# FluidInference/FluidAudio

Hardware: NVIDIA H100
Metric: audio-hours/s (higher is better)
Workload: dtype f32

## Files before the change

fluidaudio_b200/csrc/fa_common.cuh:

```cuda
#pragma once

#include <cstddef>
#include <cstdint>

#if defined(__CUDACC__)
#include <atomic>
#include <cstdio>
#include <memory>
#include <type_traits>
#include <utility>
#include <cuda_runtime.h>
#define FA_HD __host__ __device__ __forceinline__
#else
#define FA_HD inline
#endif

enum : int {
    FA_OK = 0,
    FA_INVALID_ARGUMENT = 1,
    FA_INDEX_OVERFLOW = 2,
    FA_OUTPUT_TOO_SMALL = 3,
    FA_ALLOCATION_FAILURE = 4,
    FA_RUNTIME_ERROR = 5,
    FA_NO_DEVICE = 6,
    FA_CUDA_ERROR = 7,
    FA_UNSUPPORTED = 8,
    FA_UNKNOWN_ERROR = 255,
};

namespace fa {

void set_error(const char *fmt, ...);
const char *last_error();

struct Carver {
    char *base = nullptr;
    size_t off = 0;
    template <typename T> T *take(size_t count) {
        off = (off + 255) & ~size_t(255);
        T *p = reinterpret_cast<T *>(base + off);
        off += count * sizeof(T);
        return p;
    }
};

#if defined(__CUDACC__)
struct CudaStatus {
    int code;
    template <typename T> operator T() const { return static_cast<T>(code); }
};
inline CudaStatus cuda_failure(cudaError_t e, const char *expr, const char *file, int line) {
    set_error("%s failed: %s (%s:%d)", expr, cudaGetErrorString(e), file, line);
    (void)cudaGetLastError();
    return CudaStatus{e == cudaErrorMemoryAllocation ? FA_ALLOCATION_FAILURE : FA_CUDA_ERROR};
}
#define FA_CUDA_TRY(expr)                                                                 \
    do {                                                                                  \
        const cudaError_t e__ = (expr);                                                   \
        if (e__ != cudaSuccess) return fa::cuda_failure(e__, #expr, __FILE__, __LINE__); \
    } while (0)

template <bool Pinned> struct CudaFree {
    void operator()(void *p) const { Pinned ? cudaFreeHost(p) : cudaFree(p); }
};

template <typename T, bool Pinned> class GrowBuffer {
  public:
    GrowBuffer() = default;
    GrowBuffer(GrowBuffer &&o) noexcept : p_(std::move(o.p_)), cap_(std::exchange(o.cap_, 0)) {}
    GrowBuffer &operator=(GrowBuffer &&o) noexcept {
        p_ = std::move(o.p_);
        cap_ = std::exchange(o.cap_, 0);
        return *this;
    }
    int grow(size_t bytes) {
        if (bytes <= cap_) return FA_OK;
        p_.reset();
        cap_ = 0;
        void *q = nullptr;
        const cudaError_t e = Pinned ? cudaMallocHost(&q, bytes) : cudaMalloc(&q, bytes);
        if (e != cudaSuccess) {
            char what[64];
            std::snprintf(what, sizeof(what), "%s(%zu bytes)", Pinned ? "cudaMallocHost" : "cudaMalloc", bytes);
            return cuda_failure(e, what, __FILE__, __LINE__);
        }
        p_.reset(q);
        cap_ = bytes;
        return FA_OK;
    }
    T *data() const { return static_cast<T *>(p_.get()); }
    size_t capacity() const { return cap_; }

  private:
    std::unique_ptr<void, CudaFree<Pinned>> p_;
    size_t cap_ = 0;
};
template <typename T = void> using DeviceBuffer = GrowBuffer<T, false>;
template <typename T = void> using PinnedBuffer = GrowBuffer<T, true>;

template <typename T, bool Pinned, typename Layout>
int carve_arena(GrowBuffer<T, Pinned> &buf, Layout &&layout, size_t slack = 0) {
    Carver size{nullptr};
    layout(size);
    const int st = buf.grow(size.off + slack);
    if (st != FA_OK) return st;
    Carver c{static_cast<char *>(static_cast<void *>(buf.data()))};
    layout(c);
    return FA_OK;
}

template <typename A, typename B>
int grow_slots(int slots, int grown, cudaStream_t stream, DeviceBuffer<A> &a, size_t a_slot, DeviceBuffer<B> &b,
               size_t b_slot) {
    DeviceBuffer<A> na;
    DeviceBuffer<B> nb;
    int st = na.grow((size_t)grown * a_slot * sizeof(A));
    if (st == FA_OK) st = nb.grow((size_t)grown * b_slot * sizeof(B));
    if (st != FA_OK) return st;
    if (slots) {
        FA_CUDA_TRY(cudaMemcpyAsync(na.data(), a.data(), (size_t)slots * a_slot * sizeof(A), cudaMemcpyDeviceToDevice, stream));
        FA_CUDA_TRY(cudaMemcpyAsync(nb.data(), b.data(), (size_t)slots * b_slot * sizeof(B), cudaMemcpyDeviceToDevice, stream));
        FA_CUDA_TRY(cudaStreamSynchronize(stream));
    }
    a = std::move(na);
    b = std::move(nb);
    return FA_OK;
}

struct StreamDestroy {
    void operator()(cudaStream_t s) const { cudaStreamDestroy(s); }
};
struct EventDestroy {
    void operator()(cudaEvent_t e) const { cudaEventDestroy(e); }
};
struct Stream : std::unique_ptr<std::remove_pointer_t<cudaStream_t>, StreamDestroy> {
    operator cudaStream_t() const { return get(); }
    int create(unsigned flags = cudaStreamNonBlocking) {
        cudaStream_t s = nullptr;
        FA_CUDA_TRY(cudaStreamCreateWithFlags(&s, flags));
        reset(s);
        return FA_OK;
    }
};
struct Event : std::unique_ptr<std::remove_pointer_t<cudaEvent_t>, EventDestroy> {
    operator cudaEvent_t() const { return get(); }
    int create(unsigned flags = cudaEventDefault) {
        cudaEvent_t e = nullptr;
        FA_CUDA_TRY(cudaEventCreateWithFlags(&e, flags));
        reset(e);
        return FA_OK;
    }
};

template <typename T = void> struct UploadStage {
    PinnedBuffer<T> host;
    DeviceBuffer<T> device;
    Event uploaded;
    bool in_flight = false;

    int reserve(size_t bytes) {
        if (in_flight) {
            FA_CUDA_TRY(cudaEventSynchronize(uploaded));
            in_flight = false;
        }
        const int st = device.grow(bytes);
        return st != FA_OK ? st : host.grow(bytes);
    }
    int upload(size_t bytes, cudaStream_t stream) {
        if (!uploaded) {
            const int st = uploaded.create(cudaEventDisableTiming);
            if (st != FA_OK) return st;
        }
        FA_CUDA_TRY(cudaMemcpyAsync(device.data(), host.data(), bytes, cudaMemcpyHostToDevice, stream));
        FA_CUDA_TRY(cudaEventRecord(uploaded, stream));
        in_flight = true;
        return FA_OK;
    }
};

extern std::atomic<long long> g_launches;

template <typename... Params, typename... Args>
cudaError_t launch(void (*kernel)(Params...), dim3 grid, dim3 block, size_t smem, cudaStream_t stream, Args &&...args) {
    kernel<<<grid, block, smem, stream>>>(std::forward<Args>(args)...);
    g_launches.fetch_add(1, std::memory_order_relaxed);
    return cudaGetLastError();
}

template <typename T> struct kernel_param { using type = T; };
template <typename... Params>
cudaError_t launch_cooperative(void (*kernel)(Params...), dim3 grid, dim3 block, size_t smem, cudaStream_t stream,
                               typename kernel_param<Params>::type... args) {
    void *argv[] = {&args...};
    const cudaError_t e =
        cudaLaunchCooperativeKernel(reinterpret_cast<const void *>(kernel), grid, block, argv, smem, stream);
    g_launches.fetch_add(1, std::memory_order_relaxed);
    return e != cudaSuccess ? e : cudaGetLastError();
}

inline int sm90_device_props(int dev, cudaDeviceProp &prop) {
    FA_CUDA_TRY(cudaGetDeviceProperties(&prop, dev));
    if (prop.major != 9) {
        set_error("fluidaudio_b200 requires an sm_90a device, found sm_%d%d", prop.major, prop.minor);
        return FA_NO_DEVICE;
    }
    return FA_OK;
}

__device__ __forceinline__ float2 fadd2_rn(float2 a, float2 b) { return make_float2(__fadd_rn(a.x, b.x), __fadd_rn(a.y, b.y)); }
__device__ __forceinline__ float2 fmul2_rn(float2 a, float2 b) { return make_float2(__fmul_rn(a.x, b.x), __fmul_rn(a.y, b.y)); }
__device__ __forceinline__ float2 ffma2_rn(float2 a, float2 b, float2 c) {
    return make_float2(__fmaf_rn(a.x, b.x, c.x), __fmaf_rn(a.y, b.y, c.y));
}
#endif

}
```

fluidaudio_b200/csrc/mel_kernels.cu:

```cuda
#include "mel_core.cuh"
#include "mel_plan.h"

#include <cuda_runtime.h>
#include <algorithm>
#include <cmath>
#include <vector>

namespace fa {
namespace mel {

__device__ __forceinline__ uint32_t smem_u32(const void *p) { return (uint32_t)__cvta_generic_to_shared(p); }

__device__ __forceinline__ void mbar_init(uint64_t *bar, uint32_t count) {
    asm volatile("mbarrier.init.shared::cta.b64 [%0], %1;" ::"r"(smem_u32(bar)), "r"(count));
}
__device__ __forceinline__ void mbar_expect_tx(uint64_t *bar, uint32_t bytes) {
    asm volatile("mbarrier.arrive.expect_tx.shared::cta.b64 _, [%0], %1;" ::"r"(smem_u32(bar)), "r"(bytes) : "memory");
}
__device__ __forceinline__ void mbar_arrive(uint64_t *bar) {
    asm volatile("mbarrier.arrive.shared::cta.b64 _, [%0];" ::"r"(smem_u32(bar)) : "memory");
}
__device__ __forceinline__ bool mbar_try_wait(uint64_t *bar, uint32_t parity) {
    uint32_t ok;
    asm volatile(
        "{\n\t"
        ".reg .pred p;\n\t"
        "mbarrier.try_wait.parity.shared::cta.b64 p, [%1], %2;\n\t"
        "selp.u32 %0, 1, 0, p;\n\t"
        "}"
        : "=r"(ok)
        : "r"(smem_u32(bar)), "r"(parity)
        : "memory");
    return ok != 0;
}
__device__ __forceinline__ void mbar_wait(uint64_t *bar, uint32_t parity) {
    while (!mbar_try_wait(bar, parity)) {
    }
}
__device__ __forceinline__ void bulk_g2s(void *dst, const void *src, uint32_t bytes, uint64_t *bar) {
    asm volatile("cp.async.bulk.shared::cluster.global.mbarrier::complete_tx::bytes [%0], [%1], %2, [%3];" ::"r"(
                     smem_u32(dst)),
                 "l"(src), "r"(bytes), "r"(smem_u32(bar))
                 : "memory");
}
__device__ __forceinline__ void fence_proxy_async() { asm volatile("fence.proxy.async.shared::cta;" ::: "memory"); }

struct TileGeom {
    int unit;
    long long f0;
    int nf;
    long long a0;
    long long base;
    long long gs, ge;
};

__device__ __forceinline__ const MelUnit &unit_at(const MelLaunch &P, int idx) { return P.inline_unit ? P.unit0 : P.units[idx]; }

__device__ __forceinline__ TileGeom tile_geom(const MelLaunch &P, int tile) {
    int lo = 0, hi = P.inline_unit ? 0 : P.num_units - 1;
    while (lo < hi) {
        const int mid = (lo + hi + 1) >> 1;
        if (P.units[mid].tile_begin <= tile) lo = mid; else hi = mid - 1;
    }
    const MelUnit &u = P.inline_unit ? P.unit0 : P.units[lo];
    TileGeom g;
    g.unit = lo;
    g.f0 = u.frame_begin + (long long)kTileFrames * (tile - u.tile_begin);
    const long long rem = u.frame_begin + u.frame_count - g.f0;
    g.nf = rem < kTileFrames ? (int)rem : kTileFrames;
    g.a0 = g.f0 * P.hop - P.pad;
    const long long need0 = g.a0 - 1;
    g.base = (need0 >= 0) ? (need0 & ~3LL) : -(((-need0) + 3) & ~3LL);
    long long ge = (g.a0 + P.pt_len + 3) & ~3LL;
    const long long n4 = u.n & ~3LL;
    if (ge > n4) ge = n4;
    g.gs = g.base < 0 ? 0 : g.base;
    g.ge = ge;
    if (!P.use_tma) g.ge = g.gs;
    return g;
}

struct TileInfo {
    TileGeom g;
    long long audio_off, n, out_off, out_stride;
    float last;
    int pad_;
};
__device__ __forceinline__ void make_tile_info(const MelLaunch &P, int tile, TileInfo &ti) {
    ti.g = tile_geom(P, tile);
    const MelUnit &u = unit_at(P, ti.g.unit);
    ti.audio_off = u.audio_off;
    ti.n = u.n;
    ti.out_off = u.out_off;
    ti.out_stride = u.out_stride;
    ti.last = u.last;
}

template <int kWarps, typename V, int kLayout>
__global__ void __launch_bounds__(kWarps * 32, 2) mel512_kernel(const MelLaunch P) {
    constexpr int kF = vtraits<V>::kFrames;
    extern __shared__ __align__(128) unsigned char smem[];
    float *raw0 = reinterpret_cast<float *>(smem);
    float *raw1 = raw0 + P.raw_cap;
    float *ptile = raw1 + P.raw_cap;
    cpxv<V> *fftbuf = reinterpret_cast<cpxv<V> *>(ptile + P.pt_cap);
    float *power = reinterpret_cast<float *>(fftbuf + kWarps * kFftPad);
    float *otile = power + (kTileFrames / 2) * kPairStride;
    const int ot_stride = P.ot_stride;
    float *fbw = otile + kTileFrames * ot_stride;
    int4 *fbmeta = reinterpret_cast<int4 *>(fbw + P.fb_cap);
    uint64_t *bars = reinterpret_cast<uint64_t *>(fbmeta + P.n_slots);
    TileInfo *tinfo = reinterpret_cast<TileInfo *>(bars + 2);

    const int tid = threadIdx.x, lane = tid & 31, warp = tid >> 5;

    if (tid == 0) {
        mbar_init(&bars[0], 1);
        mbar_init(&bars[1], 1);
        asm volatile("fence.mbarrier_init.release.cluster;" ::: "memory");
    }
    for (int i = tid; i < P.fb_nnz; i += kWarps * 32) fbw[i] = P.fb_w[i];
    for (int i = tid; i < P.n_slots; i += kWarps * 32) fbmeta[i] = P.fb_slots[i];
    for (int i = tid; i < (kTileFrames / 2) * kPairStride; i += kWarps * 32) power[i] = 0.0f;
    const LaneTables<V> T = reinterpret_cast<const LaneTables<V> *>(P.lane_tab)[lane];
    __syncthreads();

    cpxv<V> *buf = fftbuf + warp * kFftPad;

    auto issue = [&](int tile, int buf, TileInfo &slot) {
        make_tile_info(P, tile, slot);
        const TileGeom &g = slot.g;
        float *dst = buf ? raw1 : raw0;
        if (g.ge > g.gs) {
            const uint32_t bytes = (uint32_t)((g.ge - g.gs) * 4);
            mbar_expect_tx(&bars[buf], bytes);
            bulk_g2s(dst + (g.gs - g.base), P.audio + slot.audio_off + g.gs, bytes, &bars[buf]);
        } else {
            mbar_arrive(&bars[buf]);
        }
    };

    auto preemphasize = [&](const TileInfo &u, const float *raw) {
        const TileGeom &g = u.g;
        const float a = P.preemph;
        const bool interior = g.a0 >= 1 && g.a0 - 1 >= g.gs && g.a0 + P.pt_len <= g.ge && g.a0 + P.pt_len <= u.n;
        if (interior) {
            const float *src = raw + (g.a0 - g.base);
            if (((g.a0 - g.base) & 3) == 0 && (P.pt_len & 3) == 0) {
                const float4 *s4 = reinterpret_cast<const float4 *>(src);
                float4 *d4 = reinterpret_cast<float4 *>(ptile);
                for (int q = tid; q < (P.pt_len >> 2); q += kWarps * 32) {
                    const float4 x = s4[q];
                    float4 y = x;
                    const float prev = src[4 * q - 1];
                    if (a != 0.0f) {
                        y.x = preemph_rest(x.x, prev, a);
                        y.y = preemph_rest(x.y, x.x, a);
                        y.z = preemph_rest(x.z, x.y, a);
                        y.w = preemph_rest(x.w, x.z, a);
                    }
                    d4[q] = y;
                }
            } else if (a == 0.0f) {
                for (int t = tid; t < P.pt_len; t += kWarps * 32) ptile[t] = src[t];
            } else {
                for (int t = tid; t < P.pt_len; t += kWarps * 32) ptile[t] = preemph_rest(src[t], src[t - 1], a);
            }
        } else {
            const float *gaudio = P.audio + u.audio_off;
            auto sample = [&](long long i) -> float {
                if (i >= g.gs && i < g.ge) return raw[i - g.base];
                if (i < 0) return u.last;
                return __ldg(gaudio + i);
            };
            for (int t = tid; t < P.pt_len; t += kWarps * 32) {
                const long long i = g.a0 + t;
                float v = 0.0f;
                if (i >= 0 && i < u.n) {
                    const float x = sample(i);
                    if (a == 0.0f) v = x;
                    else if (i == 0) v = preemph_first(x, u.last, a);
                    else v = preemph_rest(x, sample(i - 1), a);
                }
                ptile[t] = v;
            }
        }
    };
    auto copy_out = [&](float *dst, int total) {
        if (P.out_vec4) {
            float4 *d4 = reinterpret_cast<float4 *>(dst);
            for (int q = tid; q < (total >> 2); q += kWarps * 32) {
                const int e = 4 * q;
                const int row = (int)__umulhi((unsigned)e, P.inv_n_mels);
                d4[q] = *reinterpret_cast<const float4 *>(otile + e + 4 * row);
            }
        } else {
            const int row_pad = ot_stride - P.n_mels;
            for (int idx = tid; idx < total; idx += kWarps * 32) {
                const int fi = P.n_mels == 1 ? idx : (int)__umulhi((unsigned)idx, P.inv_n_mels);
                dst[idx] = otile[idx + fi * row_pad];
            }
        }
    };

    const int first = blockIdx.x, stride = gridDim.x;
    if (first >= P.total_tiles) return;
    if (tid == 0) {
        issue(first, 0, tinfo[0]);
        if (first + stride < P.total_tiles) issue(first + stride, 1, tinfo[1]);
    }
    __syncthreads();
    mbar_wait(&bars[0], 0);
    preemphasize(tinfo[0], raw0);
    __syncthreads();
    float *pending_dst = nullptr;
    int pending_total = 0;
    int it = 0, slot = 0;
    for (int tile = first; tile < P.total_tiles; tile += stride, ++it, slot = slot == 2 ? 0 : slot + 1) {
        const TileInfo &u = tinfo[slot];
        const int nf = u.g.nf;

        if (pending_dst) copy_out(pending_dst, pending_total);
        for (int fi = warp * kF; fi < nf; fi += kWarps * kF) {
            const float *pf = ptile + fi * P.hop;
            V re[8], im[8];
            if (P.mid_full) pass1<true>(lane, pf, P.hop, T, buf); else pass1<false>(lane, pf, P.hop, T, buf);
            __syncwarp();
            pass2_load(lane, buf, re, im);
            __syncwarp();
            pass2_store(lane, T, re, im, buf);
            __syncwarp();
            pass3_post(lane, buf, T, power + (fi >> 1) * kPairStride + (fi & 1));
            __syncwarp();
        }
        __syncthreads();

        const int next = tile + stride;
        const int slot1 = slot == 2 ? 0 : slot + 1, slot2 = slot1 == 2 ? 0 : slot1 + 1;
        if (tid == 0 && next + stride < P.total_tiles) {
            fence_proxy_async();
            issue(next + stride, it & 1, tinfo[slot2]);
        }
        {
            constexpr int kPairs = kTileFrames / 2, kGroup = 32 / kPairs;
            const int pl = lane % kPairs, mg = lane / kPairs;
            const float *prow = power + pl * kPairStride;
            float *orow = otile + (2 * pl) * ot_stride;
            float *gout = kLayout == 1 ? P.out + u.out_off + u.g.f0 + 2 * pl : nullptr;
            for (int slot = warp * kGroup + mg; slot < P.n_slots; slot += kWarps * kGroup) {
                const int4 md = fbmeta[slot];
                const float2 a2 = mel_dot_pairs(reinterpret_cast<const float4 *>(prow + 2 * md.x),
                                                reinterpret_cast<const float4 *>(fbw + md.z), md.y);
                const float v0 = log_value(a2.x, P.log_floor, P.log_clamped, P.log_normal),
                            v1 = log_value(a2.y, P.log_floor, P.log_clamped, P.log_normal);
                const int m = md.w;
                if (m < 0) continue;
                if (kLayout == 0) {
                    orow[m] = v0;
                    orow[ot_stride + m] = v1;
                } else {
                    float *g = gout + (long long)m * u.out_stride;
                    if (2 * pl < nf) g[0] = v0;
                    if (2 * pl + 1 < nf) g[1] = v1;
                }
            }
        }
        if (kLayout == 0) {
            pending_dst = P.out + u.out_off + u.g.f0 * P.n_mels;
            pending_total = nf * P.n_mels;
        }
        if (next < P.total_tiles) {
            const int nb = (it + 1) & 1;
            mbar_wait(&bars[nb], (uint32_t)((it + 1) >> 1) & 1u);
            preemphasize(tinfo[slot1], nb ? raw1 : raw0);
        }
        __syncthreads();
    }
    if (pending_dst) copy_out(pending_dst, pending_total);
}


struct GenericParams {
    int n_fft, log2n, bins, prow;
    const cpxd *tw;
    int warps;
    float spectrum_power;
    float log_mean, log_std;
};

template <bool kReflect, int kSpectrum, bool kAffine>
__global__ void __launch_bounds__(256) mel_generic_kernel(const MelLaunch P, const GenericParams G) {
    extern __shared__ __align__(16) unsigned char smem[];
    cpxd *tw = reinterpret_cast<cpxd *>(smem);
    cpxd *fft = tw + G.n_fft / 2;
    float *power = reinterpret_cast<float *>(fft + (size_t)G.warps * G.n_fft);
    float *win = power + (size_t)G.warps * G.prow;
    const int tid = threadIdx.x, lane = tid & 31, warp = tid >> 5, nthreads = G.warps * 32;
    for (int i = tid; i < G.n_fft / 2; i += nthreads) tw[i] = G.tw[i];
    for (int i = tid; i < G.n_fft; i += nthreads) win[i] = P.in_tab[i] ? P.win_tab[i] : 0.0f;
    for (int i = tid; i < G.warps * G.prow; i += nthreads) power[i] = 0.0f;
    __syncthreads();
    cpxd *buf = fft + (size_t)warp * G.n_fft;
    float *prow = power + (size_t)warp * G.prow;
    const float a = P.preemph;
    for (int tile = blockIdx.x; tile < P.total_tiles; tile += gridDim.x) {
        const TileGeom g = tile_geom(P, tile);
        const MelUnit u = unit_at(P, g.unit);
        const float *x = P.audio + u.audio_off;
        for (int fi = warp; fi < g.nf; fi += G.warps) {
            const long long f = g.f0 + fi;
            const long long base = f * P.hop - P.pad;
            for (int j = lane; j < G.n_fft; j += 32) {
                const long long i = base + j;
                float v = 0.0f;
                if (kReflect) {
                    if (u.n > 0 && P.in_tab[j]) v = __fmul_rn(__ldg(x + reflect_index(i, u.n)), win[j]);
                } else if (i >= 0 && i < u.n && P.in_tab[j]) {
                    const float xi = __ldg(x + i);
                    if (a == 0.0f) v = xi;
                    else if (i == 0) v = preemph_first(xi, u.last, a);
                    else v = preemph_rest(xi, __ldg(x + i - 1), a);
                    v = __fmul_rn(v, win[j]);
                }
                cpxd z;
                z.x = (double)v;
                z.y = 0.0;
                buf[__brev((unsigned)j) >> (32 - G.log2n)] = z;
            }
            __syncwarp();
            for (int s = 0; s < G.log2n; ++s) {
                const int half = 1 << s, step = G.n_fft >> (s + 1);
                for (int t = lane; t < G.n_fft / 2; t += 32) {
                    const int j = t & (half - 1);
                    const int ia = ((t >> s) << (s + 1)) + j, ib = ia + half;
                    const cpxd w = tw[j * step], zb = buf[ib], za = buf[ia];
                    const double tr = zb.x * w.x - zb.y * w.y, ti = zb.x * w.y + zb.y * w.x;
                    cpxd o;
                    o.x = za.x - tr;
                    o.y = za.y - ti;
                    buf[ib] = o;
                    o.x = za.x + tr;
                    o.y = za.y + ti;
                    buf[ia] = o;
                }
                __syncwarp();
            }
            for (int b = lane; b < G.bins; b += 32) {
                const float xr = (float)buf[b].x, xi = (float)buf[b].y;
                const float pw = __fadd_rn(__fmul_rn(xr, xr), __fmul_rn(xi, xi));
                if (kSpectrum == kSpecPower) prow[b] = 4.0f * pw;
                else if (kSpectrum == kSpecMagnitude) prow[b] = __fsqrt_rn(pw);
                else prow[b] = powf(__fsqrt_rn(pw), G.spectrum_power);
            }
            __syncwarp();
            for (int m = lane; m < P.n_mels; m += 32) {
                const int lo = P.fb_lo[m], nq = (P.fb_hi[m] - lo) >> 2;
                float v = log_value(mel_dot_quads(reinterpret_cast<const float4 *>(prow + lo),
                                                  reinterpret_cast<const float4 *>(P.fb_w + P.fb_off[m]), nq),
                                    P.log_floor, P.log_clamped);
                if (kAffine) v = __fdiv_rn(__fsub_rn(v, G.log_mean), G.log_std);
                if (P.layout == 0) P.out[u.out_off + f * P.n_mels + m] = v;
                else P.out[u.out_off + (long long)m * u.out_stride + f] = v;
            }
            __syncwarp();
        }
    }
}

static constexpr int kCtasPerSm = 2;

typedef void (*Mel512Kernel)(const MelLaunch);
template <typename V> static Mel512Kernel mel512_variant(int layout) {
    return layout == FA_MEL_TIME_MAJOR ? mel512_kernel<kWarpsPerCta, V, FA_MEL_TIME_MAJOR>
                                       : mel512_kernel<kWarpsPerCta, V, FA_MEL_MEL_MAJOR>;
}
static Mel512Kernel mel512_variant(int precision, int layout) {
    return precision == FA_MEL_PRECISION_F64 ? mel512_variant<double>(layout) : mel512_variant<f32x2>(layout);
}

typedef void (*GenericKernel)(const MelLaunch, const GenericParams);
template <bool R, int S> static GenericKernel generic_variant(bool affine) {
    return affine ? mel_generic_kernel<R, S, true> : mel_generic_kernel<R, S, false>;
}
template <bool R> static GenericKernel generic_variant(int spectrum, bool affine) {
    return spectrum == kSpecPower ? generic_variant<R, kSpecPower>(affine)
                                  : (spectrum == kSpecMagnitude ? generic_variant<R, kSpecMagnitude>(affine)
                                                                : generic_variant<R, kSpecGeneral>(affine));
}
static GenericKernel generic_variant(bool reflect, int spectrum, bool affine) {
    return reflect ? generic_variant<true>(spectrum, affine) : generic_variant<false>(spectrum, affine);
}

static int placement_of(int mode) { return mode == FA_MEL_LEGACY_COMPUTE ? 1 : 0; }
static int window_offset(const MelConfig &c, int placement) { return placement == 1 ? 0 : (c.n_fft - c.win_length) / 2; }

static_assert(sizeof(MelSlot) == sizeof(int4) && offsetof(MelSlot, mel) == offsetof(int4, w), "MelSlot is an int4");

template <typename T, typename U> static int upload_table(DeviceBuffer<T> &b, const std::vector<U> &v) {
    const int st = b.grow(std::max<size_t>(1, v.size()) * sizeof(U));
    if (st != FA_OK) return st;
    if (!v.empty()) FA_CUDA_TRY(cudaMemcpy(b.data(), v.data(), v.size() * sizeof(U), cudaMemcpyHostToDevice));
    return FA_OK;
}

int MelPlan::init(const MelConfig &c) {
    cfg = c;
    if (cfg.pad_to < 1) cfg.pad_to = 1;
    if (cfg.n_mels <= 0 || cfg.hop_length <= 0 || cfg.win_length <= 0 || cfg.n_fft <= 0 || cfg.sample_rate <= 0) {
        fa::set_error("mel config: all sizes must be positive");
        return FA_INVALID_ARGUMENT;
    }
    const bool pow2 = cfg.n_fft >= 32 && cfg.n_fft <= 4096 && (cfg.n_fft & (cfg.n_fft - 1)) == 0;
    if (!pow2 || cfg.win_length > cfg.n_fft || cfg.n_mels > 512 || cfg.hop_length > 65536) {
        fa::set_error("mel config unsupported by the sm_90a kernels: need nFFT a power of two in 32..4096, win <= nFFT, "
                      "nMels <= 512 (got nFFT=%d hop=%d win=%d nMels=%d)",
                      cfg.n_fft, cfg.hop_length, cfg.win_length, cfg.n_mels);
        return FA_UNSUPPORTED;
    }
    if (const char *why = check_ex_config(cfg)) {
        fa::set_error("mel ex config: %s", why);
        return FA_INVALID_ARGUMENT;
    }
    const int spectrum = spectrum_kind(cfg.spectrum_power);
    generic = cfg.n_fft != kNfft || (cfg.hop_length & 1) || cfg.hop_length > 1024 || cfg.reflect() ||
              spectrum != kSpecPower || cfg.affine();
    const int n_fft = cfg.n_fft, bins = n_fft / 2 + 1;
    build_tables(cfg, window, filterbank);
    const MelBands bands = pack_bands(filterbank, cfg.n_mels, bins);
    fb_nnz = bands.nnz;
    n_slots = (int)bands.slots.size();

    int dev = 0;
    FA_CUDA_TRY(cudaGetDevice(&dev));
    cudaDeviceProp prop;
    int st = sm90_device_props(dev, prop);
    if (st != FA_OK) return st;
    num_sms = prop.multiProcessorCount;

    if (!generic) {
        pt_len = (kTileFrames - 1) * cfg.hop_length + kNfft;
        pt_cap = (pt_len + 31) & ~31;
        raw_cap = (pt_len + 1 + 3 + 3 + 31) & ~31;
        fb_cap = (fb_nnz + 3) & ~3;
        smem_bytes = sizeof(float) * ((size_t)2 * raw_cap + pt_cap + 0 +
                                      (size_t)(kTileFrames / 2) * kPairStride + (size_t)kTileFrames * (cfg.n_mels + 4) + fb_cap) +
                     sizeof(cpxd) * (size_t)kWarpsPerCta * kFftPad + sizeof(int) * 4 * (size_t)n_slots + 8 +
                     2 * sizeof(uint64_t) + 3 * sizeof(TileInfo) + 16;
        if (smem_bytes > (size_t)prop.sharedMemPerBlockOptin) {
            generic = true;
            pt_len = pt_cap = raw_cap = fb_cap = 0;
        }
    }

    std::vector<float> win_tab;
    std::vector<uint8_t> in_tab;
    for (int pl = 0; pl < 2; ++pl) {
        place_window(window, n_fft, window_offset(cfg, pl), win_tab, in_tab);
        st = upload_table(d_win_tab_mode[pl], win_tab);
        if (st == FA_OK) st = upload_table(d_in_tab_mode[pl], in_tab);
        if (st != FA_OK) return st;
        if (!generic) {
            std::vector<LaneTables<double>> t64(32);
            std::vector<LaneTables<f32x2>> t32(32);
            for (int l = 0; l < 32; ++l) {
                load_lane_tables(l, win_tab.data(), in_tab.data(), t64[l]);
                load_lane_tables(l, win_tab.data(), in_tab.data(), t32[l]);
            }
            st = upload_table(d_lane_tab[pl][FA_MEL_PRECISION_F64], t64);
            if (st == FA_OK) st = upload_table(d_lane_tab[pl][FA_MEL_PRECISION_F32], t32);
            if (st != FA_OK) return st;
        }
    }
    st = upload_table(d_fb_w, pack_weights(filterbank, bands, bins, !generic, spectrum == kSpecPower ? 0.25f : 1.0f));
    if (st == FA_OK) st = upload_table(d_fb_slots, bands.slots);
    if (st == FA_OK) st = upload_table(d_fb_lo, bands.lo);
    if (st == FA_OK) st = upload_table(d_fb_hi, bands.hi);
    if (st == FA_OK) st = upload_table(d_fb_off, bands.off);
    for (auto &s : streams)
        if (st == FA_OK) st = s.create();
    if (st != FA_OK) return st;
    if (generic) {
        std::vector<cpxd> tw(n_fft / 2);
        for (int k = 0; k < n_fft / 2; ++k) tw[k] = unit_root(k, n_fft);
        st = upload_table(d_generic_tw, tw);
        if (st != FA_OK) return st;
        generic_prow = ((bins + 3) & ~3) + 4;
        int log2n = 0;
        while ((1 << log2n) < n_fft) ++log2n;
        generic_log2n = log2n;
        const size_t fixed = (size_t)(n_fft / 2) * sizeof(cpxd) + (size_t)n_fft * sizeof(float);
        const size_t per_warp = (size_t)n_fft * sizeof(cpxd) + (size_t)generic_prow * sizeof(float);
        generic_warps = (int)std::min<size_t>(8, ((size_t)prop.sharedMemPerBlockOptin - fixed - 1024) / per_warp);
        if (generic_warps < 1) {
            fa::set_error("mel config: nFFT %d does not fit shared memory", n_fft);
            return FA_UNSUPPORTED;
        }
        smem_bytes = fixed + per_warp * generic_warps;
        for (const bool r : {false, cfg.reflect()})
            FA_CUDA_TRY(cudaFuncSetAttribute(generic_variant(r, spectrum, cfg.affine()),
                                             cudaFuncAttributeMaxDynamicSharedMemorySize, (int)smem_bytes));
        return FA_OK;
    }
    for (const int precision : {FA_MEL_PRECISION_F64, FA_MEL_PRECISION_F32})
        for (const int layout : {FA_MEL_TIME_MAJOR, FA_MEL_MEL_MAJOR})
            FA_CUDA_TRY(cudaFuncSetAttribute(mel512_variant(precision, layout), cudaFuncAttributeMaxDynamicSharedMemorySize,
                                             (int)smem_bytes));
    return FA_OK;
}

long long MelPlan::frame_count(long long n, int mode, long long expected) const {
    long long computed;
    if (mode == FA_MEL_PAD_CENTER) computed = 1 + (n + 2 * (long long)(cfg.n_fft / 2) - cfg.win_length) / cfg.hop_length;
    else if (mode == FA_MEL_PAD_PREPADDED) computed = std::max<long long>(0, (n - cfg.n_fft) / cfg.hop_length + 1);
    else computed = 1 + (n - cfg.win_length) / cfg.hop_length;
    return expected >= 0 ? expected : computed;
}

int MelPlan::ensure_staging(size_t audio_floats, size_t out_floats) {
    const int st = d_audio.grow(audio_floats * sizeof(float));
    return st != FA_OK ? st : d_out.grow(out_floats * sizeof(float));
}

int MelPlan::ensure_events(size_t count) {
    while (events.size() < count) {
        Event e;
        const int st = e.create(cudaEventDisableTiming);
        if (st != FA_OK) return st;
        events.push_back(std::move(e));
    }
    return FA_OK;
}

static int tiles_of(long long frames) { return (int)((frames + kTileFrames - 1) / kTileFrames); }

int number_tiles(MelUnit *u, int count) {
    int tiles = 0;
    for (int i = 0; i < count; ++i) {
        u[i].tile_begin = tiles;
        tiles += tiles_of(u[i].frame_count);
    }
    return tiles;
}

int MelPlan::launch(const MelUnit *d_u, const MelUnit *h_u, int count, bool inline_unit, const float *d_audio_base,
                    float *d_out_base, int mode, int layout, cudaStream_t stream) {
    const int total_tiles = count > 0 ? h_u[count - 1].tile_begin + tiles_of(h_u[count - 1].frame_count) : 0;
    if (total_tiles <= 0) return FA_OK;
    MelLaunch P{};
    P.audio = d_audio_base;
    P.out = d_out_base;
    P.units = d_u;
    P.num_units = count;
    P.inline_unit = (inline_unit && count == 1) ? 1 : 0;
    if (P.inline_unit) P.unit0 = h_u[0];
    P.total_tiles = total_tiles;
    P.hop = cfg.hop_length;
    P.pad = mode == FA_MEL_PAD_CENTER ? cfg.n_fft / 2 : 0;
    P.preemph = mode == FA_MEL_LEGACY_COMPUTE ? 0.0f : cfg.preemph;
    P.n_mels = cfg.n_mels;
    P.log_floor = cfg.log_floor;
    P.log_clamped = cfg.log_floor_mode;
    P.ot_stride = (cfg.n_mels & 3) == 0 ? cfg.n_mels + 4 : cfg.n_mels + 1;
    P.out_vec4 = (cfg.n_mels & 3) == 0 && (reinterpret_cast<uintptr_t>(d_out_base) & 15) == 0;
    for (int i = 0; i < count && P.out_vec4; ++i) P.out_vec4 = (h_u[i].out_off & 3) == 0;
    P.log_normal = cfg.log_floor >= 1e-37f ? 1 : 0;
    P.layout = layout;
    const int pl = placement_of(mode);
    P.lane_tab = d_lane_tab[pl][precision == FA_MEL_PRECISION_F32 ? 1 : 0].data();
    P.win_tab = d_win_tab_mode[pl].data();
    P.in_tab = d_in_tab_mode[pl].data();
    P.fb_w = d_fb_w.data();
    P.fb_slots = d_fb_slots.data();
    P.n_slots = n_slots;
    P.fb_lo = d_fb_lo.data();
    P.fb_hi = d_fb_hi.data();
    P.fb_off = d_fb_off.data();
    P.fb_nnz = fb_nnz;
    P.fb_cap = fb_cap;
    P.pt_len = pt_len;
    P.pt_cap = pt_cap;
    P.raw_cap = raw_cap;
    P.use_tma = (reinterpret_cast<uintptr_t>(d_audio_base) & 15) == 0;
    for (int i = 0; i < count && P.use_tma; ++i) P.use_tma = (h_u[i].audio_off & 3) == 0;
    {
        const int off_w = window_offset(cfg, pl);
        P.mid_full = (off_w <= 64 && off_w + cfg.win_length >= 448) ? 1 : 0;
    }
    P.inv_n_mels = (unsigned)((0x100000000ull + (unsigned)cfg.n_mels - 1) / (unsigned)cfg.n_mels);
    if (generic) {
        GenericParams G{cfg.n_fft, generic_log2n, cfg.n_fft / 2 + 1, generic_prow,
                        static_cast<const cpxd *>(d_generic_tw.data()), generic_warps, cfg.spectrum_power, cfg.log_mean,
                        cfg.log_std};
        const int ggrid = std::min(total_tiles, num_sms * std::max(1, 16 / generic_warps));
        const GenericKernel kernel = generic_variant(mode == FA_MEL_PAD_CENTER && cfg.reflect(),
                                                     spectrum_kind(cfg.spectrum_power), cfg.affine());
        FA_CUDA_TRY(fa::launch(kernel, ggrid, generic_warps * 32, smem_bytes, stream, P, G));
        return FA_OK;
    }
    const int grid = std::min(total_tiles, num_sms * kCtasPerSm);
    const dim3 blk(kWarpsPerCta * 32);
    FA_CUDA_TRY(fa::launch(mel512_variant(precision, layout), grid, blk, smem_bytes, stream, P));
    return FA_OK;
}

static bool shape_of(const MelPlan &p, long long n, int mode, long long expected, long long &T, long long &Tp) {
    T = p.frame_count(n, mode, mode == FA_MEL_PAD_CENTER || mode == FA_MEL_PAD_PREPADDED ? expected : -1);
    if (T <= 0 || n <= 0) return false;
    Tp = mode == FA_MEL_LEGACY_COMPUTE ? T : ceil_to(T, p.cfg.pad_to);
    return true;
}

int clip_shape(const MelPlan &p, long long n, int mode, long long expected, long long out_len, long long &T,
               long long &Tp, long long *mel_length, long long *num_frames) {
    if (!shape_of(p, n, mode, expected, T, Tp)) {
        T = 0;
        Tp = mode == FA_MEL_LEGACY_COMPUTE ? 0 : 1;
    }
    if (mel_length) *mel_length = T;
    if (num_frames) *num_frames = Tp;
    if (out_len < Tp * p.cfg.n_mels) {
        fa::set_error("mel output needs %lld floats, buffer has %lld", Tp * p.cfg.n_mels, out_len);
        return FA_OUTPUT_TOO_SMALL;
    }
    return FA_OK;
}

int MelPlan::compute_device(const float *d_in, long long n, float last, int mode, long long expected, int layout,
                            float *d_out_buf, long long out_len, long long *mel_length, long long *num_frames,
                            cudaStream_t stream) {
    long long T, Tp;
    int st = clip_shape(*this, n, mode, expected, out_len, T, Tp, mel_length, num_frames);
    if (st != FA_OK) return st;
    if (T == 0) {
        if (Tp) FA_CUDA_TRY(cudaMemsetAsync(d_out_buf, 0, cfg.n_mels * sizeof(float), stream));
        return FA_OK;
    }
    st = units.reserve(unit_bytes(1));
    if (st != FA_OK) return st;
    if (Tp > T) FA_CUDA_TRY(cudaMemsetAsync(d_out_buf, 0, Tp * cfg.n_mels * sizeof(float), stream));
    units.host.data()[0] = MelUnit{0, n, 0, Tp, 0, T, last, 0};
    st = units.upload(sizeof(MelUnit), stream);
    if (st != FA_OK) return st;
    return launch(units.device.data(), units.host.data(), 1, false, d_in, d_out_buf, mode, layout, stream);
}

int MelPlan::launch_clip(const float *d_in, long long n, long long T, int layout, float *d_out_buf, cudaStream_t stream) {
    if (T <= 0) return FA_OK;
    int st = units.reserve(unit_bytes(1));
    if (st != FA_OK) return st;
    units.host.data()[0] = MelUnit{0, n, 0, T, 0, T, 0.0f, 0};
    st = units.upload(sizeof(MelUnit), stream);
    if (st != FA_OK) return st;
    return launch(units.device.data(), units.host.data(), 1, false, d_in, d_out_buf, FA_MEL_PAD_CENTER, layout, stream);
}

int MelPlan::compute_batch_device(const float *d_in, const long long *offsets, int count, const float *last, int mode,
                                  int layout, float *d_out_buf, const long long *out_offsets, long long *mel_lengths,
                                  long long *num_frames, cudaStream_t stream) {
    int st = units.reserve(unit_bytes(count));
    if (st != FA_OK) return st;
    MelUnit *h_units = units.host.data();
    int used = 0;
    for (int i = 0; i < count; ++i) {
        const long long n = offsets[i + 1] - offsets[i];
        long long T, Tp;
        clip_shape(*this, n, mode, -1, kUnchecked, T, Tp, mel_lengths ? mel_lengths + i : nullptr,
                   num_frames ? num_frames + i : nullptr);
        if (T == 0) {
            if (Tp) FA_CUDA_TRY(cudaMemsetAsync(d_out_buf + out_offsets[i], 0, cfg.n_mels * sizeof(float), stream));
            continue;
        }
        if (Tp > T) FA_CUDA_TRY(cudaMemsetAsync(d_out_buf + out_offsets[i], 0, Tp * cfg.n_mels * sizeof(float), stream));
        h_units[used++] = MelUnit{offsets[i], n, out_offsets[i], Tp, 0, T, last ? last[i] : 0.0f, 0};
    }
    if (!used) return FA_OK;
    number_tiles(h_units, used);
    st = units.upload(used * sizeof(MelUnit), stream);
    if (st != FA_OK) return st;
    return launch(units.device.data(), h_units, used, false, d_in, d_out_buf, mode, layout, stream);
}

}
}
```

Measured before the change: 3114.

## Enable programmatic dependent launch for mel kernel and inline single-unit params

Launches the mel512 kernel with programmatic stream serialization so its prologue (barrier init, smem setup) can overlap the tail of the preceding kernel, gating real work on griddepcontrol.wait. For single-clip paths, it also drops the pinned-buffer unit upload and event record and passes the unit inline, using the launch function's inline flag. This reduces per-call launch latency and host-to-device copies, but it relies on the kernel correctly waiting before it reads any data the previous kernel produced.

```diff
diff --git a/fluidaudio_b200/csrc/fa_common.cuh b/fluidaudio_b200/csrc/fa_common.cuh
--- a/fluidaudio_b200/csrc/fa_common.cuh
+++ b/fluidaudio_b200/csrc/fa_common.cuh
@@ -187,6 +187,28 @@
     return cudaGetLastError();
 }
 
+template <typename... Params, typename... Args>
+cudaError_t launch_overlapped(void (*kernel)(Params...), dim3 grid, dim3 block, size_t smem, cudaStream_t stream,
+                              Args &&...args) {
+    cudaLaunchAttribute attr[1];
+    attr[0].id = cudaLaunchAttributeProgrammaticStreamSerialization;
+    attr[0].val.programmaticStreamSerializationAllowed = 1;
+    cudaLaunchConfig_t cfg = {};
+    cfg.gridDim = grid;
+    cfg.blockDim = block;
+    cfg.dynamicSmemBytes = smem;
+    cfg.stream = stream;
+    cfg.attrs = attr;
+    cfg.numAttrs = 1;
+    const cudaError_t e = cudaLaunchKernelEx(&cfg, kernel, std::forward<Args>(args)...);
+    g_launches.fetch_add(1, std::memory_order_relaxed);
+    return e != cudaSuccess ? e : cudaGetLastError();
+}
+#if defined(__CUDACC__)
+__device__ __forceinline__ void grid_dependency_wait() { asm volatile("griddepcontrol.wait;" ::: "memory"); }
+__device__ __forceinline__ void grid_launch_dependents() { asm volatile("griddepcontrol.launch_dependents;" ::: "memory"); }
+#endif
+
 template <typename T> struct kernel_param { using type = T; };
 template <typename... Params>
 cudaError_t launch_cooperative(void (*kernel)(Params...), dim3 grid, dim3 block, size_t smem, cudaStream_t stream,
diff --git a/fluidaudio_b200/csrc/mel_kernels.cu b/fluidaudio_b200/csrc/mel_kernels.cu
--- a/fluidaudio_b200/csrc/mel_kernels.cu
+++ b/fluidaudio_b200/csrc/mel_kernels.cu
@@ -113,6 +113,7 @@
     TileInfo *tinfo = reinterpret_cast<TileInfo *>(bars + 2);
 
     const int tid = threadIdx.x, lane = tid & 31, warp = tid >> 5;
+    grid_launch_dependents();
 
     if (tid == 0) {
         mbar_init(&bars[0], 1);
@@ -205,6 +206,7 @@
 
     const int first = blockIdx.x, stride = gridDim.x;
     if (first >= P.total_tiles) return;
+    grid_dependency_wait();
     if (tid == 0) {
         issue(first, 0, tinfo[0]);
         if (first + stride < P.total_tiles) issue(first + stride, 1, tinfo[1]);
@@ -599,7 +601,7 @@
     }
     const int grid = std::min(total_tiles, num_sms * kCtasPerSm);
     const dim3 blk(kWarpsPerCta * 32);
-    FA_CUDA_TRY(fa::launch(mel512_variant(precision, layout), grid, blk, smem_bytes, stream, P));
+    FA_CUDA_TRY(fa::launch_overlapped(mel512_variant(precision, layout), grid, blk, smem_bytes, stream, P));
     return FA_OK;
 }
 
@@ -635,23 +637,15 @@
         if (Tp) FA_CUDA_TRY(cudaMemsetAsync(d_out_buf, 0, cfg.n_mels * sizeof(float), stream));
         return FA_OK;
     }
-    st = units.reserve(unit_bytes(1));
-    if (st != FA_OK) return st;
     if (Tp > T) FA_CUDA_TRY(cudaMemsetAsync(d_out_buf, 0, Tp * cfg.n_mels * sizeof(float), stream));
-    units.host.data()[0] = MelUnit{0, n, 0, Tp, 0, T, last, 0};
-    st = units.upload(sizeof(MelUnit), stream);
-    if (st != FA_OK) return st;
-    return launch(units.device.data(), units.host.data(), 1, false, d_in, d_out_buf, mode, layout, stream);
+    const MelUnit u{0, n, 0, Tp, 0, T, last, 0};
+    return launch(nullptr, &u, 1, true, d_in, d_out_buf, mode, layout, stream);
 }
 
 int MelPlan::launch_clip(const float *d_in, long long n, long long T, int layout, float *d_out_buf, cudaStream_t stream) {
     if (T <= 0) return FA_OK;
-    int st = units.reserve(unit_bytes(1));
-    if (st != FA_OK) return st;
-    units.host.data()[0] = MelUnit{0, n, 0, T, 0, T, 0.0f, 0};
-    st = units.upload(sizeof(MelUnit), stream);
-    if (st != FA_OK) return st;
-    return launch(units.device.data(), units.host.data(), 1, false, d_in, d_out_buf, FA_MEL_PAD_CENTER, layout, stream);
+    const MelUnit u{0, n, 0, T, 0, T, 0.0f, 0};
+    return launch(nullptr, &u, 1, true, d_in, d_out_buf, FA_MEL_PAD_CENTER, layout, stream);
 }
 
 int MelPlan::compute_batch_device(const float *d_in, const long long *offsets, int count, const float *last, int mode,
```

New measurement: 3184, median of 6. 2.3% higher.
